# pocokhc/simple_distributed_rl

Measured on AMD Instinct MI355X. Metric: env-steps/sec + learner updates/sec, Rainbow 84x84x4, higher is better.
Workload: dtype f32

## Files before the change

### include/srlx.h

```cpp
#ifndef SRLX_H
#define SRLX_H

#include <stdint.h>

#ifdef __cplusplus
extern "C" {
#endif

#define SRLX_VERSION 1

#define SRLX_OK 0
#define SRLX_ERR_INVALID (-1)
#define SRLX_ERR_HIP (-2)
#define SRLX_ERR_NOMEM (-3)
#define SRLX_ERR_UNIFORMS_EXHAUSTED (-4)
#define SRLX_ERR_UNSUPPORTED (-5)

const char *srlx_last_error(void);
int srlx_version(void);
int srlx_stream_create(int priority_level, void **out_stream);
int srlx_stream_destroy(void *stream);
int srlx_debug_stamp(uint64_t *d_buf, int index, void *stream);
int srlx_device_count(int *out_count);
int srlx_device_info(int device, char *arch_name, int arch_name_len, int *cu_count, int64_t *hbm_bytes);
// ... 294 lines not shown

int srlx_store_obs_base(srlx_store_t *h, void **d_base, int64_t *frame_bytes);
int srlx_store_locate(srlx_store_t *h, int64_t batch, const int64_t *d_tree_idx, int64_t *d_env, int64_t *d_slot, int64_t *d_prev_slot, void *stream);
int srlx_store_frame_table_current(srlx_store_t *h, int64_t *d_out, void *stream);
int srlx_store_gather_items(srlx_store_t *h, int64_t batch, const int64_t *d_tree_idx, int k_begin, int k_count, int64_t *d_frame_off,
                            int32_t *d_actions, float *d_rewards, float *d_terminated, void *stream);
int srlx_store_gather_train(srlx_store_t *h, int64_t batch, const int64_t *d_tree_idx, int64_t *d_frame_off_all, int64_t *d_frame_off_next,
                            int32_t *d_actions, float *d_rewards, float *d_terminated, void *stream);
int srlx_per_sample_gather_train(srlx_per_t *h, srlx_store_t *store, int64_t batch_size, const int64_t *d_step, uint64_t seed, int64_t *d_counter, int64_t n_uniforms,
                                 int64_t *d_out_idx, float *d_out_w32, int64_t *d_out_used, int64_t *d_frame_off_all, int64_t *d_frame_off_next, int32_t *d_actions,
                                 float *d_rewards, float *d_terminated, void *stream);
int srlx_store_actor_td(srlx_store_t *h, int64_t first_slot, int64_t per_capacity, const float *d_q_hist, int base_slot, const uint8_t *d_item_mask, double discount,
                        double retrace_h, int enable_double_dqn, int enable_rescale, float *d_est, void *stream);
int srlx_store_gather_obs(srlx_store_t *h, int64_t batch, int k_begin, int k_count, float *d_obs, void *stream);

typedef struct srlx_qnet srlx_qnet_t;
int srlx_qnet_create(srlx_qnet_t **out, int in_h, int in_w, int window, int filters, int hidden, int n_actions, int dueling_type, int64_t max_batch,
                     int device);
int srlx_qnet_destroy(srlx_qnet_t *h);
int srlx_qnet_bind(srlx_qnet_t *h, const float *const *d_params);
int srlx_qnet_forward_u8(srlx_qnet_t *h, int64_t batch, const uint8_t *d_frame_base, const int64_t *d_frame_off, float *d_q, void *stream);
int srlx_qnet_forward_u8_policy(srlx_qnet_t *h, int64_t batch, const uint8_t *d_frame_base, const int64_t *d_frame_off, float *d_q, const float *d_eps, uint64_t seed,
                                const int64_t *d_counter, const uint8_t *d_invalid, int32_t *d_actions, float *d_q_copy, void *stream);
int srlx_qnet_actor_sets_enable(srlx_qnet_t *h);
int srlx_qnet_actor_set_planes(srlx_qnet_t *h, int set, void **d_planes);
int srlx_qnet_actor_set_select(srlx_qnet_t *h, int set);
int srlx_qnet_publish(srlx_qnet_t *h_src, srlx_qnet_t *h_actor, int set, int with_fc1, int64_t *d_bump, void *stream);
int srlx_qnet_set_priority_sink(srlx_qnet_t *h, srlx_per_t *per, int64_t n, const int64_t *d_indices, const void *d_priorities, int prio_kind);
int srlx_qnet_set_sink_wait(srlx_qnet_t *h, void *event);
int srlx_qnet_set_sink_done(srlx_qnet_t *h, void *event);
int srlx_qnet_set_sink_stream(srlx_qnet_t *h, void *stream);
int srlx_qnet_set_main_first(srlx_qnet_t *h, int on);
int srlx_qnet_set_dgrad_split(srlx_qnet_t *h, int splits);

int srlx_qnet_set_td_event(srlx_qnet_t *h, void *event);
int srlx_qnet_set_stamp_buffer(srlx_qnet_t *h, uint64_t *d_buf);
int srlx_qnet_set_fc1_branch(srlx_qnet_t *h, int order);
int srlx_qnet_fuse_adam_fc1_planes(srlx_qnet_t *h, void *d_planes_out);
int srlx_qnet_set_pack_sticky(srlx_qnet_t *h, int on);
int srlx_qnet_set_fc1_neighbour(srlx_qnet_t *h, int splits);
int srlx_qnet_set_planes_small(srlx_qnet_t *h, int on, const void *d_weight_planes);
int srlx_qnet_weights_changed(srlx_qnet_t *h);
int srlx_qnet_forward_convs_u8(srlx_qnet_t *h, int64_t batch, const uint8_t *d_frame_base, const int64_t *d_frame_off, float *d_features, void *stream);
int srlx_qnet_set_probe(srlx_qnet_t *h, void *ev_start, void *ev_end);
int srlx_qnet_set_probe_fc1(srlx_qnet_t *h, void *ev_start, void *ev_end);
int srlx_qnet_set_fc1_span(srlx_qnet_t *h, uint64_t *d_span);
int srlx_qnet_enable_fc1_planes(srlx_qnet_t *h);
int srlx_qnet_refresh_fc1_planes(srlx_qnet_t *h, const float *d_src_wf, float *d_copy_dst, void *stream);
int srlx_qnet_invalidate_fc1_planes(srlx_qnet_t *h);
int srlx_qnet_set_debug(srlx_qnet_t *h, void *d_phase_stamps);
int srlx_qnet_range_flags(srlx_qnet_t *h, int *out_bits);
int srlx_qnet_enable_training(srlx_qnet_t *h, int64_t max_train_batch);
int srlx_qnet_fuse_adam_fc1(srlx_qnet_t *h, float *d_exp_avg, float *d_exp_avg_sq, double lr, double beta1, double beta2, double eps,
                            const int64_t *d_steps_taken);
int srlx_qnet_fuse_adam_rest(srlx_qnet_t *h, const float *const *d_grads, float *const *d_exp_avg, float *const *d_exp_avg_sq);
int srlx_qnet_backward_u8(srlx_qnet_t *h, int64_t batch, int64_t sample_stride, const uint8_t *d_frame_base, const int64_t *d_frame_off,
                          const float *d_grad_q, float *const *d_grads, void *stream);
int srlx_qnet_backward_convs_u8(srlx_qnet_t *h, int64_t batch, int64_t sample_stride, const uint8_t *d_frame_base, const int64_t *d_frame_off,
                                const float *d_grad_features, float *const *d_grads, void *stream);
int srlx_qnet_backward_td_u8(srlx_qnet_t *h, int64_t batch, int n_step, const uint8_t *d_frame_base, const int64_t *d_frame_off, const float *d_q_on_all,
                             const float *d_q_tg_next, const int32_t *d_actions, const float *d_rewards, const float *d_terminated,
                             const uint8_t *d_invalid_next, const float *d_weights, double discount, double retrace_h, int enable_double_dqn,
                             int enable_rescale, float *d_target, float *d_loss, float *d_grad_q0, float *d_priorities, float *const *d_grads, void *stream);
int srlx_qnet_forward_f32(srlx_qnet_t *h, int64_t batch, const float *d_obs_nchw, float *d_q, void *stream);
int srlx_qnet_forward_convs_multi_u8(srlx_qnet_t *const *hs, int n, int64_t batch, const uint8_t *d_frame_base, const int64_t *d_frame_off, void *stream);
int srlx_qnet_forward_dense_planes(srlx_qnet_t *h, int64_t batch, float *d_q, void *stream);
// ... 71 lines not shown
```

### simple_distributed_rl_amd/_native.py

```python
import ctypes
import os
import threading

_HERE = os.path.dirname(os.path.abspath(__file__))
LIB_PATH = os.environ.get("SRLX_LIB") or os.path.join(_HERE, "libsrlx.so")

os.environ.setdefault("GPU_MAX_HW_QUEUES", "2")

OK = 0
ERR_INVALID, ERR_HIP, ERR_NOMEM, ERR_UNIFORMS_EXHAUSTED, ERR_UNSUPPORTED = -1, -2, -3, -4, -5
PRIO_NONE, PRIO_F64, PRIO_F32, PRIO_RAW = 0, 1, 2, 3

c_i64 = ctypes.c_int64
c_f64 = ctypes.c_double
c_u64 = ctypes.c_uint64
c_int = ctypes.c_int
c_p = ctypes.c_void_p


class SrlxError(RuntimeError):
    def __init__(self, status, message):
        super().__init__(f"libsrlx error {status}: {message}")
        self.status = status

# ... 50 lines not shown
    "srlx_store_views": (c_int, [c_p, ctypes.POINTER(c_p), ctypes.POINTER(c_p), ctypes.POINTER(c_p)]),
    "srlx_store_gather_nstep": (c_int, [c_p, c_i64, c_p, c_p, c_p, c_p, c_p, c_p]),
    "srlx_store_locate": (c_int, [c_p, c_i64, c_p, c_p, c_p, c_p, c_p]),
    "srlx_agent57_ucb_step": (c_int, [c_i64, c_int, c_int, c_p, c_p, c_p, c_p, c_p, c_p, c_p, c_p, c_p, c_p, c_f64, c_f64, c_p]),
    "srlx_store_obs_base": (c_int, [c_p, ctypes.POINTER(c_p), ctypes.POINTER(c_i64)]),
    "srlx_store_frame_table_current": (c_int, [c_p, c_p, c_p]),
    "srlx_store_gather_items": (c_int, [c_p, c_i64, c_p, c_int, c_int, c_p, c_p, c_p, c_p, c_p]),
    "srlx_store_gather_train": (c_int, [c_p, c_i64, c_p, c_p, c_p, c_p, c_p, c_p, c_p]),
    "srlx_store_gather_obs": (c_int, [c_p, c_i64, c_int, c_int, c_p, c_p]),
    "srlx_qnet_create": (c_int, [ctypes.POINTER(c_p), c_int, c_int, c_int, c_int, c_int, c_int, c_int, c_i64, c_int]),
    "srlx_qnet_destroy": (c_int, [c_p]),
    "srlx_qnet_bind": (c_int, [c_p, c_p]),
    "srlx_qnet_forward_u8": (c_int, [c_p, c_i64, c_p, c_p, c_p, c_p]),
    "srlx_qnet_forward_convs_multi_u8": (c_int, [c_p, c_int, c_i64, c_p, c_p, c_p]),
    "srlx_qnet_forward_dense_planes": (c_int, [c_p, c_i64, c_p, c_p]),
    "srlx_qnet_forward_convs_u8": (c_int, [c_p, c_i64, c_p, c_p, c_p, c_p]),
    "srlx_qnet_forward_u8_policy": (c_int, [c_p, c_i64, c_p, c_p, c_p, c_p, c_u64, c_p, c_p, c_p, c_p, c_p]),
    "srlx_qnet_actor_sets_enable": (c_int, [c_p]),
    "srlx_qnet_actor_set_planes": (c_int, [c_p, c_int, ctypes.POINTER(c_p)]),
    "srlx_qnet_actor_set_select": (c_int, [c_p, c_int]),
    "srlx_qnet_publish": (c_int, [c_p, c_p, c_int, c_int, c_p, c_p]),
    "srlx_debug_stamp": (c_int, [c_p, c_int, c_p]),
    "srlx_stream_create": (c_int, [c_int, ctypes.POINTER(c_p)]),
    "srlx_stream_destroy": (c_int, [c_p]),
    "srlx_qnet_set_fc1_branch": (c_int, [c_p, c_int]),
    "srlx_qnet_set_stamp_buffer": (c_int, [c_p, c_p]),
    "srlx_qnet_set_td_event": (c_int, [c_p, c_p]),
    "srlx_qnet_set_priority_sink": (c_int, [c_p, c_p, c_i64, c_p, c_p, c_int]),
    "srlx_qnet_set_sink_wait": (c_int, [c_p, c_p]),
    "srlx_qnet_set_sink_done": (c_int, [c_p, c_p]),
    "srlx_qnet_set_sink_stream": (c_int, [c_p, c_p]),
    "srlx_qnet_set_main_first": (c_int, [c_p, c_int]),
    "srlx_qnet_set_dgrad_split": (c_int, [c_p, c_int]),
    "srlx_qnet_fuse_adam_fc1_planes": (c_int, [c_p, c_p]),
    "srlx_qnet_set_pack_sticky": (c_int, [c_p, c_int]),
    "srlx_qnet_set_fc1_neighbour": (c_int, [c_p, c_int]),
    "srlx_qnet_set_planes_small": (c_int, [c_p, c_int, c_p]),
    "srlx_qnet_weights_changed": (c_int, [c_p]),
    "srlx_qnet_enable_training": (c_int, [c_p, c_i64]),
    "srlx_qnet_set_probe": (c_int, [c_p, c_p, c_p]),
    "srlx_qnet_set_probe_fc1": (c_int, [c_p, c_p, c_p]),
    "srlx_qnet_set_fc1_span": (c_int, [c_p, c_p]),
    "srlx_qnet_enable_fc1_planes": (c_int, [c_p]),
    "srlx_qnet_refresh_fc1_planes": (c_int, [c_p, c_p, c_p, c_p]),
    "srlx_qnet_invalidate_fc1_planes": (c_int, [c_p]),
    "srlx_qnet_set_debug": (c_int, [c_p, c_p]),
    "srlx_qnet_range_flags": (c_int, [c_p, c_p]),
    "srlx_qnet_fuse_adam_fc1": (c_int, [c_p, c_p, c_p, c_f64, c_f64, c_f64, c_f64, c_p]),
    "srlx_qnet_fuse_adam_rest": (c_int, [c_p, c_p, c_p, c_p]),
    "srlx_qnet_backward_u8": (c_int, [c_p, c_i64, c_i64, c_p, c_p, c_p, c_p, c_p]),
    "srlx_qnet_backward_convs_u8": (c_int, [c_p, c_i64, c_i64, c_p, c_p, c_p, c_p, c_p]),
    "srlx_qnet_backward_td_u8": (c_int, [c_p, c_i64, c_int, c_p, c_p, c_p, c_p, c_p, c_p, c_p, c_p, c_p, c_f64, c_f64, c_int, c_int, c_p, c_p, c_p, c_p, c_p, c_p]),
    "srlx_qnet_forward_f32": (c_int, [c_p, c_i64, c_p, c_p, c_p]),
    "srlx_qnet_bind_noisy": (c_int, [c_p, c_p, c_u64]),
    "srlx_qnet_bind_noisy_grads": (c_int, [c_p, c_p]),
    "srlx_qnet_redraw_rows": (c_int, [c_p, c_i64, c_i64, c_p, c_p]),
    "srlx_qnet_noisy_effective": (c_int, [c_p, c_int, c_p, ctypes.POINTER(c_i64), ctypes.POINTER(c_i64), c_p]),
    "srlx_policy_epsilon_greedy": (c_int, [c_i64, c_int, c_p, c_p, c_p, c_p, c_p, c_p]),
    "srlx_image_preprocess": (c_int, [c_i64, c_int, c_int, c_int, c_p, c_int, c_int, c_int, c_int, c_int, c_int, c_int, c_p, c_p, c_int, c_f64, c_p]),
    "srlx_episode_account": (c_int, [c_i64, c_p, c_p, c_p, c_p, c_p, c_p, c_i64, c_p, c_p]),
    "srlx_synth_env_step": (c_int, [c_p, c_i64, c_p, c_p, c_p, c_p, c_p]),
    "srlx_synth_env_step_at": (c_int, [c_p, c_i64, c_i64, c_p, c_p, c_p, c_p, c_p]),
    "srlx_nstep_td_huber_priority": (
        c_int,
        [c_i64, c_int, c_int, c_p, c_p, c_p, c_p, c_p, c_p, c_p, c_p, c_f64, c_f64, c_int, c_int, c_p, c_p, c_p, c_p, c_p],
    ),
# ... 212 lines not shown
```

### simple_distributed_rl_amd/csrc/srlx_qnet.hip

```cpp
#include <new>

#include "srlx_qnet_int.h"

namespace {

using i64 = int64_t;
using u8 = unsigned char;
using f32x16 = __attribute__((ext_vector_type(16))) float;
using bf16x8 = __attribute__((ext_vector_type(8))) __bf16;

constexpr int BM = 128, BK = 32, LDT = 36;

__device__ __forceinline__ int clampi(int v, int lo, int hi) { return v < lo ? lo : (v > hi ? hi : v); }

struct APlain {
    const float *A;
    i64 lda;
    struct Row {
        const float *p;
    };
    __device__ __forceinline__ Row row(i64 m, i64 M) const { return Row{m < M ? A + m * lda : nullptr}; }
    __device__ __forceinline__ float4 load4(const Row &r, int k0, int c4) const {
        return r.p ? *reinterpret_cast<const float4 *>(r.p + k0 + c4) : make_float4(0.f, 0.f, 0.f, 0.f);
    }
// ... 860 lines not shown
        dim3 grid((unsigned)((M + BM - 1) / BM), 1, Z);
        hipLaunchKernelGGL((k_gemm_s16<ADgrad, 32, false>), grid, dim3(256), 0, st, a, wT, dXq, M, CI, K, K, (i64)CI * K, M * CI);
    }
    SRLX_HIP(hipGetLastError());
    return SRLX_OK;
}

extern "C" {

int srlx_qnet_create(srlx_qnet_t **out, int in_h, int in_w, int window, int filters, int hidden, int n_actions, int dueling_type, int64_t max_batch,
                     int device) {
    SRLX_REQUIRE(out, "qnet_create: out is NULL");
    SRLX_REQUIRE(in_h >= 8 && in_w >= 8 && window >= 1 && filters % 32 == 0 && hidden % 32 == 0 && n_actions >= 1 && n_actions <= kMaxActions && max_batch > 0,
                 "qnet_create: unsupported shape (filters and hidden must be multiples of 32, n_actions <= %d)", kMaxActions);
    SRLX_REQUIRE((window * 64) % BK == 0, "qnet_create: window*64 must be a multiple of %d", BK);
    SRLX_REQUIRE(filters == 32 || filters == 64 || filters == 128, "qnet_create: filters must be 32, 64 or 128 (channel counts are powers of two, <= 80 K-slabs)");
    SRLX_REQUIRE(dueling_type >= 0 && dueling_type <= kHeadPlain, "qnet_create: dueling_type 0 (average), 1 (max), 2 (naive) or 3 (plain Q head, no dueling)");
    int ndev = 0;
    SRLX_HIP(hipGetDeviceCount(&ndev));
    SRLX_REQUIRE(device >= 0 && device < ndev, "qnet_create: device %d not present", device);
    srlx::DeviceGuard guard(device);
    srlx_qnet *h = new (std::nothrow) srlx_qnet();
    if (!h) return SRLX_ERR_NOMEM;
    memset(h, 0, sizeof(*h));
    h->device = device;
    h->H = in_h, h->W = in_w, h->Wn = window, h->F1 = filters, h->hidden = hidden, h->A = n_actions, h->dueling = dueling_type;
    h->OH1 = conv_out(in_h, 8, 4, 3), h->OW1 = conv_out(in_w, 8, 4, 3);
    h->OH2 = conv_out(h->OH1, 4, 2, 2), h->OW2 = conv_out(h->OW1, 4, 2, 2);
    h->OH3 = conv_out(h->OH2, 3, 1, 1), h->OW3 = conv_out(h->OW2, 3, 1, 1);
    h->flat = h->OH3 * h->OW3 * 2 * filters;
    h->max_batch = max_batch;
    h->max_splits = 64;
    h->aset_cur = -1;
    SRLX_REQUIRE(h->flat % BK == 0, "qnet_create: flattened size %d must be a multiple of %d", h->flat, BK);
    const size_t f = sizeof(float);
    struct {
        float **p;
        size_t n;
    } bufs[] = {{&h->act1, (size_t)max_batch * h->OH1 * h->OW1 * filters},
                {&h->act2, (size_t)max_batch * h->OH2 * h->OW2 * 2 * filters},
                {&h->act3, (size_t)max_batch * h->flat},
                {&h->partial, (size_t)(4096 + 128 + max_batch) * 2 * hidden}};
    h->partial_floats = bufs[3].n;
    for (auto &b : bufs) {
        hipError_t e = hipMalloc((void **)b.p, b.n * f);
        if (e != hipSuccess) {
            srlx::set_error("qnet_create: %s", hipGetErrorString(e));
            srlx_qnet_destroy(h);
            return e == hipErrorOutOfMemory ? SRLX_ERR_NOMEM : SRLX_ERR_HIP;
        }
    }
    if (hipMalloc((void **)&h->range_flag, sizeof(int)) != hipSuccess || hipMemset(h->range_flag, 0, sizeof(int)) != hipSuccess) {
        srlx::set_error("qnet_create: the range flag");
        srlx_qnet_destroy(h);
        return SRLX_ERR_HIP;
    }
    *out = h;
    return SRLX_OK;
}

int srlx_qnet_range_flags(srlx_qnet_t *h, int *out) {
    SRLX_REQUIRE(h && out, "qnet_range_flags: NULL argument");
    srlx::DeviceGuard guard(h->device);
    SRLX_HIP(hipMemcpy(out, h->range_flag, sizeof(int), hipMemcpyDeviceToHost));
    return SRLX_OK;
}
// ... 197 lines not shown
    return SRLX_OK;
}

int srlx_qnet_set_planes_small(srlx_qnet_t *h, int on, const void *d_weight_planes) {
    SRLX_REQUIRE(h, "qnet_set_planes_small: NULL handle");
    SRLX_REQUIRE(!on || h->a3_planes, "qnet_set_planes_small: srlx_qnet_enable_fc1_planes first");
    h->planes_small = on != 0;
    h->wf_planes_ext = d_weight_planes;
    if (on && h->fc1_neighbour <= 0) h->fc1_neighbour = 4;
    if (d_weight_planes) h->planes_valid = true;
    return SRLX_OK;
}

int srlx_qnet_set_priority_sink(srlx_qnet_t *h, srlx_per_t *per, int64_t n, const int64_t *d_indices, const void *d_priorities, int prio_kind) {
    SRLX_REQUIRE(h, "qnet_set_priority_sink: NULL handle");
    SRLX_REQUIRE(!per || (h->max_train > 0 && n > 0 && d_indices && d_priorities), "qnet_set_priority_sink: enable training first; n > 0 and device pointers");
    h->sink_per = per, h->sink_n = n, h->sink_idx = d_indices, h->sink_prio = d_priorities, h->sink_kind = prio_kind;
    return SRLX_OK;
}

int srlx_qnet_set_sink_done(srlx_qnet_t *h, void *event) {
    SRLX_REQUIRE(h, "qnet_set_sink_done: NULL handle");
    h->sink_done = (hipEvent_t)event;
    return SRLX_OK;
}

int srlx_qnet_set_main_first(srlx_qnet_t *h, int on) {
    SRLX_REQUIRE(h, "qnet_set_main_first: NULL handle");
    h->main_first = on != 0;
    return SRLX_OK;
}

int srlx_qnet_set_dgrad_split(srlx_qnet_t *h, int splits) {
    SRLX_REQUIRE(h && (splits == 1 || splits == 2), "qnet_set_dgrad_split: 1 or 2");
    h->dgrad_split = splits;
    return SRLX_OK;
}

int srlx_qnet_set_sink_stream(srlx_qnet_t *h, void *stream) {
    SRLX_REQUIRE(h, "qnet_set_sink_stream: NULL handle");
    h->sink_stream = (hipStream_t)stream;
    return SRLX_OK;
}

int srlx_qnet_set_sink_wait(srlx_qnet_t *h, void *event) {
    SRLX_REQUIRE(h, "qnet_set_sink_wait: NULL handle");
    h->sink_wait = (hipEvent_t)event;
    return SRLX_OK;
}

int srlx_qnet_set_fc1_branch(srlx_qnet_t *h, int order) {
    SRLX_REQUIRE(h && order >= 0 && order <= 2, "qnet_set_fc1_branch: order 0 (last on the weight-gradient branch), 1 (first on it) or 2 (a branch of its own)");
    h->fc1_order = order;
    return SRLX_OK;
}

int srlx_qnet_set_stamp_buffer(srlx_qnet_t *h, uint64_t *d_buf) {
    SRLX_REQUIRE(h, "qnet_set_stamp_buffer: NULL handle");
    h->stamp_buf = d_buf;
    return SRLX_OK;
}

int srlx_qnet_set_td_event(srlx_qnet_t *h, void *event) {
    SRLX_REQUIRE(h, "qnet_set_td_event: NULL handle");
    h->ev_td = (hipEvent_t)event;
    return SRLX_OK;
}

int srlx_qnet_fuse_adam_fc1_planes(srlx_qnet_t *h, void *d_planes_out) {
    SRLX_REQUIRE(h, "qnet_fuse_adam_fc1_planes: NULL handle");
// ... 126 lines not shown
```

### simple_distributed_rl_amd/csrc/srlx_qnet_bwd.hip

```cpp
#include <new>

#include "srlx_adam_math.h"
#include "srlx_qnet_int.h"
#include "srlx_td_math.h"

namespace {

using i64 = int64_t;
using u8 = unsigned char;
using f32x16 = __attribute__((ext_vector_type(16))) float;

constexpr int kFcSplits = 16;
constexpr int kWgSplits = 64;
constexpr int kC1Pad = 88, kC1Frame = kC1Pad * kC1Pad, kC1Chunks = 4;

__device__ __forceinline__ int clampi(int v, int lo, int hi) { return v < lo ? lo : (v > hi ? hi : v); }
__device__ __forceinline__ float byte_to_unit(unsigned b) {
    const float x = (float)b, rcp = 1.0f / 255.0f;
    const float q = x * rcp;
    return fmaf(fmaf(-q, 255.0f, x), rcp, q);
}

template <int AMAX>
__global__ void __launch_bounds__(256) k_head_bwd(int B, i64 sstride, int hidden, int A, int dueling, const float *dq,
// ... 722 lines not shown
#define SRLX_STAMP(idx, stream) \
    if (h->stamp_buf) SRLX_TRY(srlx_debug_stamp(h->stamp_buf, (idx), (stream)))

static int chain_prologue(srlx_qnet_t *h, hipStream_t st, int part = 3, bool with_uvfa = false, int uvfa_B = 0, i64 uvfa_ss = 1) {
    hipStream_t sd = h->side;
    if (part & 1) SRLX_HIP(hipEventRecord(h->ev_fork, st));
    if (!(part & 2)) return SRLX_OK;
    SRLX_HIP(hipStreamWaitEvent(sd, h->ev_fork, 0));
    hipStream_t sk = h->sink_per && h->sink_stream ? h->sink_stream : sd;
    if (sk != sd) SRLX_HIP(hipStreamWaitEvent(sk, h->ev_fork, 0));
    if (h->sink_per && h->sink_wait) SRLX_HIP(hipStreamWaitEvent(sk, h->sink_wait, 0));
    if (h->sink_per) SRLX_TRY(srlx_per_update(h->sink_per, h->sink_n, h->sink_idx, h->sink_prio, h->sink_kind, 1, sk));
    if (h->sink_per && h->sink_done) SRLX_HIP(hipEventRecord(h->sink_done, sk));
    SRLX_STAMP(21, sd);
    if (h->uvfa.X > 0 && h->uvfa.g_wx && with_uvfa) {
        const int N1 = 2 * h->hidden;
        hipLaunchKernelGGL(k_uvfa_wgrad, dim3((unsigned)((h->uvfa.X * N1 + 255) / 256)), dim3(256), 0, sd, uvfa_B, uvfa_ss, N1, h->uvfa.X, srlx_uvfa_args(h), h->dh1, h->uvfa.g_wx);
    }
    const int C2 = 2 * h->F1;
    if (!h->wt_from_forward) {
        hipLaunchKernelGGL(k_transpose_filter, dim3((unsigned)((C2 * 9 * C2 + 255) / 256)), dim3(256), 0, st, h->w3, C2, 3, 3, 1, C2, h->w_t);
        hipLaunchKernelGGL(k_transpose_filter, dim3((unsigned)((C2 * 16 * h->F1 + 255) / 256)), dim3(256), 0, st, h->w2, C2, 4, 4, 2, h->F1, h->w_t2);
    }
    return SRLX_OK;
}

static int conv_chain(srlx_qnet_t *h, int B, i64 ss, const uint8_t *d_frame_base, const int64_t *d_frame_off, float *const *g, hipStream_t st, bool with_fc1) {
    const int N1 = 2 * h->hidden, K = h->flat, C2 = 2 * h->F1;
    float *g_w1 = g[0], *g_b1 = g[1], *g_w2 = g[2], *g_b2 = g[3], *g_w3 = g[4], *g_b3 = g[5], *g_wf = with_fc1 ? g[6] : nullptr;
    float *bias_part = h->w_part + h->w_part_floats;
    const size_t c3 = (size_t)2 * h->F1 * 9 * 2 * h->F1, c2 = (size_t)2 * h->F1 * 16 * h->F1;
    hipStream_t sd = h->side;
    SRLX_HIP(hipEventRecord(h->ev_d3, st));
    {
        const int HP = h->OH2 + 2, WP = h->OW2 + 2;
        const int nsplit = (C2 == 64 && h->dgrad_split == 2) ? 2 : 1;
        SRLX_TRY(srlx_qnet_dgrad_gemm(h->dact3, B, HP, WP, h->OH3, h->OW3, C2, 3, 3, 1, h->w_t, C2, h->dxpad, st, nsplit));
        const i64 tot = (i64)B * h->OH2 * h->OW2 * C2;
        hipLaunchKernelGGL(k_fold_pad, dim3((unsigned)((tot / 4 + 255) / 256)), dim3(256), 0, st, B, ss, h->OH2, h->OW2, C2, 1, HP, WP, 1, HP, WP, h->dxpad, h->act2, h->dact2, nsplit,
                           (i64)B * HP * WP * C2);
    }
    SRLX_STAMP(18, st);
    SRLX_HIP(hipEventRecord(h->ev_d2, st));
    {
        const int HP = h->OH1 + 4, WP = h->OW1 + 4, QH = (HP + 1) / 2, QW = (WP + 1) / 2;
        SRLX_TRY(srlx_qnet_dgrad_gemm(h->dact2, B, QH, QW, h->OH2, h->OW2, C2, 4, 4, 2, h->w_t2, h->F1, h->dxpad, st));
        const i64 tot = (i64)B * h->OH1 * h->OW1 * h->F1;
        hipLaunchKernelGGL(k_fold_pad, dim3((unsigned)((tot / 4 + 255) / 256)), dim3(256), 0, st, B, ss, h->OH1, h->OW1, h->F1, 2, HP, WP, 2, QH, QW, h->dxpad, h->act1, h->dact1);
    }
    SRLX_STAMP(19, st);
    SRLX_HIP(hipEventRecord(h->ev_d1, st));
    const dim3 fg((unsigned)((K / 32 + 3) / 4), (unsigned)(N1 / 32));
    if (with_fc1 && !h->adam_m)
        hipLaunchKernelGGL(k_fc1_wgrad<false>, fg, dim3(256), 0, sd, B, ss, N1, K, h->dh1, h->act3, g_wf, nullptr, nullptr, nullptr, 0.0, 0.0, 0.0, 0.0, nullptr);
    SRLX_HIP(hipStreamWaitEvent(sd, h->ev_d3, 0));
    const int fc1_order = h->fc1_order;
    auto launch_fc1_adam = [&](hipStream_t s2) {
        if (h->adam_planes_out)
            hipLaunchKernelGGL((k_fc1_wgrad<true, true>), fg, dim3(256), 0, s2, B, ss, N1, K, h->dh1, h->act3, nullptr, const_cast<float *>(h->wf), h->adam_m, h->adam_v,
                               h->adam_lr, h->adam_b1, h->adam_b2, h->adam_eps, h->adam_step, (_Float16 *)h->adam_planes_out);
        else
            hipLaunchKernelGGL(k_fc1_wgrad<true>, fg, dim3(256), 0, s2, B, ss, N1, K, h->dh1, h->act3, nullptr, const_cast<float *>(h->wf), h->adam_m, h->adam_v, h->adam_lr,
                               h->adam_b1, h->adam_b2, h->adam_eps, h->adam_step);
    };
    const bool fc1_adam = with_fc1 && h->adam_m;
    if (fc1_adam && fc1_order == 1) launch_fc1_adam(sd);
    if (fc1_adam && fc1_order == 2) {
        if (!h->side2) SRLX_HIP(hipStreamCreateWithFlags(&h->side2, hipStreamNonBlocking));
        SRLX_HIP(hipStreamWaitEvent(h->side2, h->ev_d3, 0));
        launch_fc1_adam(h->side2);
        SRLX_HIP(hipEventRecord(h->ev_join2, h->side2));
    }
    ConvGeo g3{h->OH2, h->OW2, C2, h->OH3, h->OW3, C2, 3, 3, 1, 1};
    hipLaunchKernelGGL(k_conv_wgrad_mfma<64>, dim3((9 * 2 * 2 + 3) / 4, (unsigned)B), dim3(256), 0, sd, g3, ss, h->act2, h->dact3, h->w_part, bias_part);
    const bool rest = h->rest_on && with_fc1;
    const AdamArgs ad{h->adam_lr, h->adam_b1, h->adam_b2, h->adam_eps, h->adam_step};
    auto reduce = [&](hipStream_t s_, const float *part_, int P_, i64 n_, float *gw_, const float *bp_, int nb_, float *gb_, int wi, i64 *snap_) {
// ... 155 lines not shown
```

### simple_distributed_rl_amd/csrc/srlx_qnet_int.h

```cpp
#pragma once
#include "srlx_common.h"

constexpr int kHeadPlain = 3;

struct srlx_qnet {
    int device;
    int H, W, Wn, F1, hidden, A, dueling;
    int OH1, OW1, OH2, OW2, OH3, OW3;
    int64_t max_batch;
    int flat;
    const float *w1, *b1, *w2, *b2, *w3, *b3, *wf, *bf, *v2w, *v2b, *a2w, *a2b;
    float *act1, *act2, *act3, *partial;
    int max_splits;
    int64_t max_train;
    float *h1;
    float *dh1, *dact3, *dact2, *dact1;
    float *fc_part;
    float *dh1t;
    float *w_part;
    float *dxpad, *w_t, *w_t2;
    size_t w_part_floats;
    hipStream_t side;
    hipEvent_t ev_fork, ev_d3, ev_d2, ev_d1, ev_join, ev_wt;
    float *adam_m, *adam_v;
// ... 94 lines not shown
    auto pad = [](int n) { return (n + 3) & ~3; };
    srlx_small_layout L;
    L.b1 = 0;
    L.b2 = L.b1 + pad(h->F1);
    L.b3 = L.b2 + pad(2 * h->F1);
    L.bf = L.b3 + pad(2 * h->F1);
    L.v2w = L.bf + pad(2 * h->hidden);
    const bool plain = h->dueling == kHeadPlain;
    L.v2b = L.v2w + (plain ? 0 : pad(h->hidden));
    L.a2w = L.v2b + (plain ? 0 : 4);
    L.a2b = L.a2w + pad(h->A * (plain ? 2 : 1) * h->hidden);
    L.wx = L.a2b + pad(h->A);
    L.total = L.wx + pad(h->uvfa.X * 2 * h->hidden);
    return L;
}

int srlx_qnet_noisy_refresh(srlx_qnet *h, hipStream_t st);
int srlx_qnet_noisy_sigma_grads(srlx_qnet *h, float *const *g, hipStream_t st);
int srlx_qnet_dense_rows(srlx_qnet *h, int64_t rows, int64_t stride, float *d_q, hipStream_t st);

bool srlx_qnet_fused_convs(srlx_qnet *h, int64_t batch, const uint8_t *d_frame_base, const int64_t *d_frame_off, hipStream_t st);

int srlx_qnet_fused_convs_multi(srlx_qnet *const *hs, int n, int64_t batch, const uint8_t *d_frame_base, const int64_t *d_frame_off, hipStream_t st);

int srlx_fc1_planes_alloc(srlx_qnet *h);
int srlx_fc1_planes_split_weight(srlx_qnet *h, const float *src, float *copy_dst, hipStream_t st, void *planes_dst = nullptr);
size_t srlx_fc1_planes_weight_bytes(const srlx_qnet *h);
int srlx_qnet_pack_publish(srlx_qnet *src, srlx_qnet::ActorSet *dst_set, const srlx_small_layout *L, hipStream_t st, int64_t *bump = nullptr, bool adam_small = false);
size_t srlx_qnet_pack_bytes();
int srlx_fc1_planes_split_act(srlx_qnet *h, int64_t rows, hipStream_t st);
bool srlx_fc1_planes_applicable(const srlx_qnet *h, int64_t rows);
int srlx_fc1_planes_gemm(srlx_qnet *h, int64_t rows, int splits, int kps, hipStream_t st);

int srlx_qnet_dgrad_gemm(const float *dY, int B, int QH, int QW, int OH, int OW, int CO, int KH, int KW, int S, const float *wT, int CI, float *dXq,
                         hipStream_t st, int ksplits = 1);
```

### simple_distributed_rl_amd/device/rainbow.py

```python
import os
from dataclasses import dataclass, field
from typing import Optional

import torch

from simple_distributed_rl_amd import _native as N
from simple_distributed_rl_amd.device import lockstep
from simple_distributed_rl_amd.device.replay import DeviceReplay
from simple_distributed_rl_amd.device.qnet import DeviceAdam, EngineQNet, QNetInference, check_ranges


@dataclass
class EngineSchedule:
    fast: Optional[bool] = None
    lagged_add: bool = True
    predraw: Optional[bool] = None
    fc1_neighbour: int = 4
    dgrad_split: Optional[int] = None
    fc1_planes: str = "auto"
    actor_stream: Optional[str] = None
    learner_priority: int = -1
    fused_adam: bool = True
    fused_adam_rest: bool = True
    fused_td: bool = True
# ... 175 lines not shown
            self.inf_actor.enable_actor_sets()
            self.inf_actor.set_fc1_neighbour(int(sch.fc1_neighbour))
        elif not self.noisy and E >= 512 and E % 128 == 0 and (2 * hid) % 128 == 0 and (planes == "1" or (planes == "auto" and not overlap)):
            self.inf_actor.enable_fc1_planes(private_weights=self.q_actor is not self.q_online)
        self.inf_online = QNetInference(self.q_online, max(B * (n + 1), 64), device, noise_seed=cfg.seed * 3 + 0x0B0E)
        self.inf_target = QNetInference(self.q_target, B * n, device, noise_seed=cfg.seed * 3 + 0x7A26)
        if self.mfma_train:
            self.inf_online.enable_training(B)
            self.s_target = torch.cuda.Stream(device=self.dev, priority=-1)
            self._ev_t0, self._ev_t1 = torch.cuda.Event(), torch.cuda.Event()
            self.optimizer = DeviceAdam(self.inf_online._params(), lr=cfg.lr)
        else:
            self.optimizer = torch.optim.Adam(self.q_online.parameters(), lr=cfg.lr, capturable=True, fused=True)
        self.actor_priority = bool(cfg.actor_initial_priority) and self.mfma
        self._init_common(cfg, E, B, A, H, W_)
        d = self.dev
        self.train_count_dev = torch.zeros(1, dtype=torch.int64, device=d)
        self._fused_td = bool(sch.fused_td)
        self.lreplay.count_updates_in(self.train_count_dev)
        if fused_adam:
            self.optimizer.fuse_first_dense(self.inf_online, self.train_count_dev)
        if self.fast:
            if role == "both":
                self._planes_ptr = [self.inf_actor.set_planes_ptr(0), self.inf_actor.set_planes_ptr(1)]
            self._set, self._published = 0, None
            self._seen_versions = None
            self.inf_target.set_pack_sticky(True)
            self._learner_planes = False
            self._fresh_set = None
            self._update_side = self._fused_td and getattr(self.lreplay, "h_per", None) is not None
            if self.actor_stream is not None and want == "low":
                N.check(self.lib.srlx_qnet_set_fc1_branch(self.inf_online.h, 2))
            N.check(self.lib.srlx_qnet_set_main_first(self.inf_online.h, 1))
            if sch.dgrad_split is None or int(sch.dgrad_split) == 2:
                N.check(self.lib.srlx_qnet_set_dgrad_split(self.inf_online.h, 2))
            if self._update_side:
                N.check(self.lib.srlx_per_set_update_counter(self.lreplay.h_per, None))
            if fused_adam and not self.noisy and sch.fused_adam_rest:
                self.optimizer.fuse_rest(self.inf_online)
            if role == "both" and learner_replay is None:
                self.replay.enable_deferred_advance()
            self._publish_out_of_band()
        self.target = torch.zeros(B, dtype=torch.float32, device=d)
        self.loss = torch.zeros(1, dtype=torch.float32, device=d)
        self.grad_q0 = torch.zeros((B, A), dtype=torch.float32, device=d)
        self.priorities = torch.zeros(B, dtype=torch.float32, device=d)
        self._learner_graphs = lockstep.UpdateGraphs(self.dev)
        self.ingest = None
        self.s_ingest = torch.cuda.Stream(device=self.dev, priority=-1) if (learner_replay is not None or self.replay.lagged) else None
        self._ev_drawn, self._ev_ingested, self._ev_sunk, self._ev_predrawn = torch.cuda.Event(), torch.cuda.Event(), torch.cuda.Event(), torch.cuda.Event()
        for ev in (self._ev_drawn, self._ev_ingested, self._ev_sunk, self._ev_predrawn):
            ev.record()
        self._predraw = bool(self.fast and self._update_side and self.s_ingest is not None and getattr(self.lreplay, "two_sets", False)
                             and (sch.predraw if sch.predraw is not None else (learner_replay is not None and role == "learner")))
        self._bset, self._drawn, self._drawn_at = 0, None, 0
        self._seen_commits, self._unnoted = 0, 0
        self.s_predraw = torch.cuda.Stream(device=self.dev, priority=-1) if self._predraw else None

    @property
    def lreplay(self) -> DeviceReplay:
        return self.learner_replay if self.learner_replay is not None else self.replay

    def _init_common(self, cfg, E, B, A, H, W_):
        d = self.dev
        if self.actor_priority:
            n1 = cfg.multisteps + 1
            self.q_hist = torch.zeros((n1, E, cfg.n_actions), dtype=torch.float32, device=d)
# ... 505 lines not shown
```

Before: 2.110 million.

## Fuse conv3 and conv2 data-gradient passes into one per-sample LDS-resident kernel

Adds a per-sample kernel that computes the conv3 and conv2 data gradients, including the col2im-style overlap sums and ReLU masks, entirely in LDS. It uses bf16x3 split MFMA to keep near-f32 accuracy. It replaces two separate dgrad GEMMs plus scatter/mask kernels and their intermediate global buffers, and becomes the default when the geometry fits. The trade-off is a large LDS footprint per block (one block per sample) and triple MFMA work for the precision emulation.

```diff
diff --git a/include/srlx.h b/include/srlx.h
--- a/include/srlx.h
+++ b/include/srlx.h
@@ -350,6 +350,7 @@
 int srlx_qnet_set_sink_stream(srlx_qnet_t *h, void *stream);
 int srlx_qnet_set_main_first(srlx_qnet_t *h, int on);
 int srlx_qnet_set_dgrad_split(srlx_qnet_t *h, int splits);
+int srlx_qnet_get_dgrad_split(const srlx_qnet_t *h);
 
 int srlx_qnet_set_td_event(srlx_qnet_t *h, void *event);
 int srlx_qnet_set_stamp_buffer(srlx_qnet_t *h, uint64_t *d_buf);
diff --git a/simple_distributed_rl_amd/_native.py b/simple_distributed_rl_amd/_native.py
--- a/simple_distributed_rl_amd/_native.py
+++ b/simple_distributed_rl_amd/_native.py
@@ -106,6 +106,7 @@
     "srlx_qnet_set_sink_stream": (c_int, [c_p, c_p]),
     "srlx_qnet_set_main_first": (c_int, [c_p, c_int]),
     "srlx_qnet_set_dgrad_split": (c_int, [c_p, c_int]),
+    "srlx_qnet_get_dgrad_split": (c_int, [c_p]),
     "srlx_qnet_fuse_adam_fc1_planes": (c_int, [c_p, c_p]),
     "srlx_qnet_set_pack_sticky": (c_int, [c_p, c_int]),
     "srlx_qnet_set_fc1_neighbour": (c_int, [c_p, c_int]),
diff --git a/simple_distributed_rl_amd/csrc/srlx_qnet.hip b/simple_distributed_rl_amd/csrc/srlx_qnet.hip
--- a/simple_distributed_rl_amd/csrc/srlx_qnet.hip
+++ b/simple_distributed_rl_amd/csrc/srlx_qnet.hip
@@ -916,6 +916,7 @@
     h->max_batch = max_batch;
     h->max_splits = 64;
     h->aset_cur = -1;
+    h->dgrad_split = 1;
     SRLX_REQUIRE(h->flat % BK == 0, "qnet_create: flattened size %d must be a multiple of %d", h->flat, BK);
     const size_t f = sizeof(float);
     struct {
@@ -1179,10 +1180,14 @@
 }
 
 int srlx_qnet_set_dgrad_split(srlx_qnet_t *h, int splits) {
-    SRLX_REQUIRE(h && (splits == 1 || splits == 2), "qnet_set_dgrad_split: 1 or 2");
+    SRLX_REQUIRE(h && splits >= 0 && splits <= 2, "qnet_set_dgrad_split: 0 (fused per-sample kernel), 1 or 2");
+    SRLX_REQUIRE(splits != 0 || srlx_qnet_dgrad_fused_covers(h), "qnet_set_dgrad_split: the fused data-gradient kernel covers 32 first-layer filters and padded grids of at most "
+                                                                  "192 rows within 160 KB of LDS, not this handle's %d x %d / %d x %d activations", h->OH1, h->OW1, h->OH2, h->OW2);
     h->dgrad_split = splits;
     return SRLX_OK;
 }
+
+int srlx_qnet_get_dgrad_split(const srlx_qnet_t *h) { return h ? h->dgrad_split : -1; }
 
 int srlx_qnet_set_sink_stream(srlx_qnet_t *h, void *stream) {
     SRLX_REQUIRE(h, "qnet_set_sink_stream: NULL handle");
diff --git a/simple_distributed_rl_amd/csrc/srlx_qnet_bwd.hip b/simple_distributed_rl_amd/csrc/srlx_qnet_bwd.hip
--- a/simple_distributed_rl_amd/csrc/srlx_qnet_bwd.hip
+++ b/simple_distributed_rl_amd/csrc/srlx_qnet_bwd.hip
@@ -778,7 +778,9 @@
     const size_t c3 = (size_t)2 * h->F1 * 9 * 2 * h->F1, c2 = (size_t)2 * h->F1 * 16 * h->F1;
     hipStream_t sd = h->side;
     SRLX_HIP(hipEventRecord(h->ev_d3, st));
-    {
+    const bool fused_dgrad = h->dgrad_split == 0;
+    if (fused_dgrad) SRLX_TRY(srlx_qnet_dgrad_fused(h, B, ss, st));
+    if (!fused_dgrad) {
         const int HP = h->OH2 + 2, WP = h->OW2 + 2;
         const int nsplit = (C2 == 64 && h->dgrad_split == 2) ? 2 : 1;
         SRLX_TRY(srlx_qnet_dgrad_gemm(h->dact3, B, HP, WP, h->OH3, h->OW3, C2, 3, 3, 1, h->w_t, C2, h->dxpad, st, nsplit));
@@ -788,7 +790,7 @@
     }
     SRLX_STAMP(18, st);
     SRLX_HIP(hipEventRecord(h->ev_d2, st));
-    {
+    if (!fused_dgrad) {
         const int HP = h->OH1 + 4, WP = h->OW1 + 4, QH = (HP + 1) / 2, QW = (WP + 1) / 2;
         SRLX_TRY(srlx_qnet_dgrad_gemm(h->dact2, B, QH, QW, h->OH2, h->OW2, C2, 4, 4, 2, h->w_t2, h->F1, h->dxpad, st));
         const i64 tot = (i64)B * h->OH1 * h->OW1 * h->F1;
diff --git a/simple_distributed_rl_amd/csrc/srlx_qnet_dgrad_fused.hip b/simple_distributed_rl_amd/csrc/srlx_qnet_dgrad_fused.hip
--- /dev/null
+++ b/simple_distributed_rl_amd/csrc/srlx_qnet_dgrad_fused.hip
@@ -0,0 +1,213 @@
+#include "srlx_qnet_int.h"
+
+namespace {
+
+using i64 = int64_t;
+using f32x16 = __attribute__((ext_vector_type(16))) float;
+using bf16x8 = __attribute__((ext_vector_type(8))) __bf16;
+using bf16x4 = __attribute__((ext_vector_type(4))) __bf16;
+
+constexpr int kWaves = 8, kC2 = 64, kF1 = 32;
+constexpr int kRow = 144;
+constexpr int kMaxTiles = 6;
+constexpr size_t kLdsMax = 160 * 1024;
+
+__device__ __forceinline__ void lds_barrier() { asm volatile("s_waitcnt lgkmcnt(0)\n\ts_barrier" ::: "memory"); }
+
+struct DgArgs {
+    int OH1, OW1, OH2, OW2;
+    int PS;
+    int o_off;
+    i64 ss;
+    const float *dact3, *act2, *act1, *wt3, *wt2;
+    float *dact2, *dact1;
+};
+
+__device__ __forceinline__ void put_parts(unsigned char *pl, int PS, int at, const float4 &x) {
+    float r[4] = {x.x, x.y, x.z, x.w};
+#pragma unroll
+    for (int p = 0; p < 3; p++) {
+        bf16x4 part;
+#pragma unroll
+        for (int j = 0; j < 4; j++) {
+            const __bf16 b = (__bf16)r[j];
+            part[j] = b;
+            r[j] -= (float)b;
+        }
+        *reinterpret_cast<bf16x4 *>(pl + p * PS + at) = part;
+    }
+}
+
+template <int KWS>
+__device__ __forceinline__ void dgrad_tiles(const unsigned char *pl, int PS, int nzero, int M, int QW, int OH, int OW, int tile0, int ntiles, const float *__restrict__ wrow,
+                                            int s0, int s1, int lane, f32x16 (&acc)[3]) {
+    const int i = lane & 31, h = lane >> 5;
+    int qy[3], qx[3];
+    bool live[3];
+#pragma unroll
+    for (int ms = 0; ms < 3; ms++) {
+        const int m = (tile0 + ms) * 32 + i;
+        live[ms] = m < M;
+        qy[ms] = m / QW, qx[ms] = m % QW;
+    }
+    float4 w0 = *reinterpret_cast<const float4 *>(wrow + s0 * 16), w1 = *reinterpret_cast<const float4 *>(wrow + s0 * 16 + 4);
+    for (int s = s0; s < s1; s++) {
+        float r[8] = {w0.x, w0.y, w0.z, w0.w, w1.x, w1.y, w1.z, w1.w};
+        if (s + 1 < s1) w0 = *reinterpret_cast<const float4 *>(wrow + (s + 1) * 16), w1 = *reinterpret_cast<const float4 *>(wrow + (s + 1) * 16 + 4);
+        bf16x8 bf[3];
+#pragma unroll
+        for (int p = 0; p < 3; p++)
+#pragma unroll
+            for (int j = 0; j < 8; j++) {
+                const __bf16 b = (__bf16)r[j];
+                bf[p][j] = b;
+                r[j] -= (float)b;
+            }
+        const int tap = s >> 2, a = tap / KWS, bq = tap - a * KWS;
+        const int off = (s & 3) * 32 + h * 16;
+        bf16x8 af[3][3];
+#pragma unroll
+        for (int ms = 0; ms < 3; ms++)
+            if (tile0 + ms < ntiles) {
+                const int oy = qy[ms] - a, ox = qx[ms] - bq;
+                const bool ok = live[ms] && oy >= 0 && ox >= 0 && oy < OH && ox < OW;
+                const unsigned char *src = pl + (ok ? oy * OW + ox : nzero) * kRow + off;
+#pragma unroll
+                for (int p = 0; p < 3; p++) af[ms][p] = *reinterpret_cast<const bf16x8 *>(src + p * PS);
+            }
+        constexpr int pq[6][2] = {{2, 0}, {0, 2}, {1, 1}, {1, 0}, {0, 1}, {0, 0}};
+#pragma unroll
+        for (int c = 0; c < 6; c++)
+#pragma unroll
+            for (int ms = 0; ms < 3; ms++)
+                if (tile0 + ms < ntiles) acc[ms] = __builtin_amdgcn_mfma_f32_32x32x16_bf16(af[ms][pq[c][0]], bf[pq[c][1]], acc[ms], 0, 0, 0);
+    }
+}
+
+__global__ void __launch_bounds__(64 * kWaves) k_conv_dgrad_fused(DgArgs g) {
+    extern __shared__ __attribute__((aligned(16))) unsigned char smem[];
+    unsigned char *pl = smem;
+    float *O = reinterpret_cast<float *>(smem + g.o_off);
+    const int t = threadIdx.x, wave = t >> 6, lane = t & 63, i = lane & 31, h = lane >> 5;
+    const i64 b = blockIdx.x;
+    const int n2 = g.OH2 * g.OW2, n1 = g.OH1 * g.OW1, nzero = n2, PS = g.PS;
+
+    {
+        const float *src = g.dact3 + b * n2 * kC2;
+        for (int idx = t; idx < n2 * 16; idx += 64 * kWaves) put_parts(pl, PS, (idx >> 4) * kRow + (idx & 15) * 8, *reinterpret_cast<const float4 *>(src + idx * 4));
+        if (t < 27) *reinterpret_cast<float4 *>(pl + (t / 9) * PS + nzero * kRow + (t % 9) * 16) = make_float4(0.f, 0.f, 0.f, 0.f);
+    }
+    lds_barrier();
+
+    const int HP3 = g.OH2 + 2, WP3 = g.OW2 + 2, M3 = HP3 * WP3, T3 = (M3 + 31) / 32;
+    {
+        const int nt = wave & 1, kh = (wave >> 1) & 1, tile0 = (wave >> 2) * 3;
+        f32x16 acc[3];
+#pragma unroll
+        for (int ms = 0; ms < 3; ms++)
+#pragma unroll
+            for (int r = 0; r < 16; r++) acc[ms][r] = 0.f;
+        if (tile0 < T3) dgrad_tiles<3>(pl, PS, nzero, M3, WP3, g.OH2, g.OW2, tile0, T3, g.wt3 + (i64)(nt * 32 + i) * (9 * kC2) + 8 * h, kh * 18, kh * 18 + 18, lane, acc);
+        if (kh == 1)
+#pragma unroll
+            for (int ms = 0; ms < 3; ms++)
+#pragma unroll
+                for (int r = 0; r < 16; r++) {
+                    const int m = (tile0 + ms) * 32 + (r & 3) + 8 * (r >> 2) + 4 * h;
+                    if (m < M3) O[m * kC2 + nt * 32 + i] = acc[ms][r];
+                }
+        lds_barrier();
+        if (kh == 0)
+#pragma unroll
+            for (int ms = 0; ms < 3; ms++)
+#pragma unroll
+                for (int r = 0; r < 16; r++) {
+                    const int m = (tile0 + ms) * 32 + (r & 3) + 8 * (r >> 2) + 4 * h;
+                    if (m < M3) O[m * kC2 + nt * 32 + i] = acc[ms][r] + O[m * kC2 + nt * 32 + i];
+                }
+    }
+    lds_barrier();
+
+    for (int idx = t; idx < n2 * 16; idx += 64 * kWaves) {
+        const int ci = (idx & 15) * 4, pix = idx >> 4, iy = pix / g.OW2, ix = pix % g.OW2;
+        const int y0 = iy == 0 ? 0 : iy + 1, y1 = iy == g.OH2 - 1 ? HP3 - 1 : iy + 1;
+        const int x0 = ix == 0 ? 0 : ix + 1, x1 = ix == g.OW2 - 1 ? WP3 - 1 : ix + 1;
+        float4 s = make_float4(0.f, 0.f, 0.f, 0.f);
+        for (int py = y0; py <= y1; py++)
+            for (int px = x0; px <= x1; px++) {
+                const float4 v = *reinterpret_cast<const float4 *>(O + (py * WP3 + px) * kC2 + ci);
+                s.x += v.x, s.y += v.y, s.z += v.z, s.w += v.w;
+            }
+        const float4 x = *reinterpret_cast<const float4 *>(g.act2 + (b * g.ss * n2 + pix) * kC2 + ci);
+        const float4 d = make_float4(x.x > 0.f ? s.x : 0.f, x.y > 0.f ? s.y : 0.f, x.z > 0.f ? s.z : 0.f, x.w > 0.f ? s.w : 0.f);
+        *reinterpret_cast<float4 *>(g.dact2 + (b * n2 + pix) * kC2 + ci) = d;
+        put_parts(pl, PS, pix * kRow + ci * 2, d);
+    }
+    lds_barrier();
+
+    const int HP2 = g.OH1 + 4, WP2 = g.OW1 + 4, QH = (HP2 + 1) / 2, QW = (WP2 + 1) / 2, M2 = QH * QW, T2 = (M2 + 31) / 32;
+    {
+        const int cls = wave & 3, tile0 = (wave >> 2) * 3;
+        f32x16 acc[3];
+#pragma unroll
+        for (int ms = 0; ms < 3; ms++)
+#pragma unroll
+            for (int r = 0; r < 16; r++) acc[ms][r] = 0.f;
+        if (tile0 < T2) dgrad_tiles<2>(pl, PS, nzero, M2, QW, g.OH2, g.OW2, tile0, T2, g.wt2 + (i64)(cls * kF1 + i) * (4 * kC2) + 8 * h, 0, 16, lane, acc);
+#pragma unroll
+        for (int ms = 0; ms < 3; ms++)
+#pragma unroll
+            for (int r = 0; r < 16; r++) {
+                const int m = (tile0 + ms) * 32 + (r & 3) + 8 * (r >> 2) + 4 * h;
+                if (m < M2) O[(cls * M2 + m) * kF1 + i] = acc[ms][r];
+            }
+    }
+    lds_barrier();
+
+    for (int idx = t; idx < n1 * 8; idx += 64 * kWaves) {
+        const int ci = (idx & 7) * 4, pix = idx >> 3, iy = pix / g.OW1, ix = pix % g.OW1;
+        const int y0 = iy == 0 ? 0 : iy + 2, y1 = iy == g.OH1 - 1 ? HP2 - 1 : iy + 2;
+        const int x0 = ix == 0 ? 0 : ix + 2, x1 = ix == g.OW1 - 1 ? WP2 - 1 : ix + 2;
+        float4 s = make_float4(0.f, 0.f, 0.f, 0.f);
+        for (int py = y0; py <= y1; py++)
+            for (int px = x0; px <= x1; px++) {
+                const float4 v = *reinterpret_cast<const float4 *>(O + ((((py & 1) * 2 + (px & 1)) * M2) + (py >> 1) * QW + (px >> 1)) * kF1 + ci);
+                s.x += v.x, s.y += v.y, s.z += v.z, s.w += v.w;
+            }
+        const float4 x = *reinterpret_cast<const float4 *>(g.act1 + (b * g.ss * n1 + pix) * kF1 + ci);
+        *reinterpret_cast<float4 *>(g.dact1 + (b * n1 + pix) * kF1 + ci) =
+            make_float4(x.x > 0.f ? s.x : 0.f, x.y > 0.f ? s.y : 0.f, x.z > 0.f ? s.z : 0.f, x.w > 0.f ? s.w : 0.f);
+    }
+}
+
+struct DgLayout {
+    int PS, o_off;
+    size_t total;
+};
+DgLayout dg_layout(const srlx_qnet *h) {
+    DgLayout L{0, 0, 0};
+    if (h->F1 != kF1 || h->OH3 != h->OH2 || h->OW3 != h->OW2) return L;
+    const int M3 = (h->OH2 + 2) * (h->OW2 + 2), M2 = ((h->OH1 + 5) / 2) * ((h->OW1 + 5) / 2);
+    if (M3 > 32 * kMaxTiles || M2 > 32 * kMaxTiles) return L;
+    L.PS = (h->OH2 * h->OW2 + 1) * kRow;
+    L.o_off = 3 * L.PS;
+    const size_t o3 = (size_t)M3 * kC2 * sizeof(float), o2 = (size_t)4 * M2 * kF1 * sizeof(float);
+    const size_t total = (size_t)L.o_off + (o3 > o2 ? o3 : o2);
+    if (total <= kLdsMax) L.total = total;
+    return L;
+}
+
+}
+
+bool srlx_qnet_dgrad_fused_covers(const srlx_qnet *h) { return dg_layout(h).total > 0; }
+
+int srlx_qnet_dgrad_fused(srlx_qnet *h, int B, int64_t ss, hipStream_t st) {
+    const DgLayout L = dg_layout(h);
+    SRLX_REQUIRE(L.total > 0, "qnet_dgrad_fused: geometry not covered");
+    static const hipError_t attr = hipFuncSetAttribute((const void *)k_conv_dgrad_fused, hipFuncAttributeMaxDynamicSharedMemorySize, (int)kLdsMax);
+    SRLX_HIP(attr);
+    DgArgs g{h->OH1, h->OW1, h->OH2, h->OW2, L.PS, L.o_off, ss, h->dact3, h->act2, h->act1, h->w_t, h->w_t2, h->dact2, h->dact1};
+    hipLaunchKernelGGL(k_conv_dgrad_fused, dim3((unsigned)B), dim3(64 * kWaves), L.total, st, g);
+    SRLX_HIP(hipGetLastError());
+    return SRLX_OK;
+}
diff --git a/simple_distributed_rl_amd/csrc/srlx_qnet_int.h b/simple_distributed_rl_amd/csrc/srlx_qnet_int.h
--- a/simple_distributed_rl_amd/csrc/srlx_qnet_int.h
+++ b/simple_distributed_rl_amd/csrc/srlx_qnet_int.h
@@ -150,5 +150,8 @@
 bool srlx_fc1_planes_applicable(const srlx_qnet *h, int64_t rows);
 int srlx_fc1_planes_gemm(srlx_qnet *h, int64_t rows, int splits, int kps, hipStream_t st);
 
+bool srlx_qnet_dgrad_fused_covers(const srlx_qnet *h);
+int srlx_qnet_dgrad_fused(srlx_qnet *h, int B, int64_t ss, hipStream_t st);
+
 int srlx_qnet_dgrad_gemm(const float *dY, int B, int QH, int QW, int OH, int OW, int CO, int KH, int KW, int S, const float *wT, int CI, float *dXq,
                          hipStream_t st, int ksplits = 1);
diff --git a/simple_distributed_rl_amd/device/rainbow.py b/simple_distributed_rl_amd/device/rainbow.py
--- a/simple_distributed_rl_amd/device/rainbow.py
+++ b/simple_distributed_rl_amd/device/rainbow.py
@@ -231,7 +231,9 @@
             if self.actor_stream is not None and want == "low":
                 N.check(self.lib.srlx_qnet_set_fc1_branch(self.inf_online.h, 2))
             N.check(self.lib.srlx_qnet_set_main_first(self.inf_online.h, 1))
-            if sch.dgrad_split is None or int(sch.dgrad_split) == 2:
+            if sch.dgrad_split is None and self.lib.srlx_qnet_set_dgrad_split(self.inf_online.h, 0) == 0:
+                pass
+            elif sch.dgrad_split is None or int(sch.dgrad_split) == 2:
                 N.check(self.lib.srlx_qnet_set_dgrad_split(self.inf_online.h, 2))
             if self._update_side:
                 N.check(self.lib.srlx_per_set_update_counter(self.lreplay.h_per, None))
```

After: 1.876 million. 0.889x the previous value.
